# benjisu03/grayshift

Hardware: AMD Instinct MI355X
Metric: Msamples/sec (primary+secondary rays) (higher is better)
Workload: dtype f64; 1 GPU; C4: bouncing_spheres_50 1920x1080, 512 spp; tile=64, parallelism=tiles1, tile_plan=round-robin, collective=none, launch=one process, 1 device(s): gs_multi_create once, gs_multi_render per frame, seed=1, rays_per_frame=2921120250

## Files before the change

__graft_entry__.py:

```python
import os
import sys

ROOT = os.path.dirname(os.path.abspath(__file__))


def build():
    sys.path.insert(0, ROOT)
    from grayshift_amd import build as b
    b.build_product()
    b.build_oracle()
    b.build_kat()
    import grayshift_amd
    from grayshift_amd import _native


def smoke():
    sys.path.insert(0, ROOT)
    sys.path.insert(0, os.path.join(ROOT, "oracle"))
    import numpy as np
    import grayshift_amd as g
    from grayshift_amd import scenes
    import oracle

    sc = scenes.config("C4", width=48, spp=4)
    out, gc = g.render(sc, seed=7)
    ref, rc = oracle.render(sc, seed=7)
    d = float(np.abs(out.astype(np.float64) - ref.astype(np.float64)).max())
    if not (d < 1e-3) or gc != rc:
        raise AssertionError("smoke parity failed: max|d|=%g counters gpu=%s oracle=%s" % (d, gc, rc))
    print("smoke ok: C4 48x27x4spp max|d|=%g rays=%d" % (d, gc["rays"]))


if __name__ == "__main__":
    build()
# ... 3 lines not shown
```

grayshift_amd/build.py:

```python
import argparse
import glob
import os
import subprocess
import sys

HERE = os.path.dirname(os.path.abspath(__file__))
ROOT = os.path.dirname(HERE)
LIB = os.path.join(HERE, "libgrayshift.so")
ORACLE_DIR = os.path.join(ROOT, "oracle")
ORACLE_LIB = os.path.join(ORACLE_DIR, "liboracle.so")

SOURCES = [
    os.path.join(HERE, "csrc", "device", "render.hip"),
    os.path.join(HERE, "csrc", "device", "output.hip"),
    os.path.join(HERE, "csrc", "device", "bvh_build.hip"),
    os.path.join(HERE, "csrc", "host", "scene.cpp"),
    os.path.join(HERE, "csrc", "host", "launch.cpp"),
    os.path.join(HERE, "csrc", "host", "world.cpp"),
    os.path.join(HERE, "csrc", "host", "camera.cpp"),
    os.path.join(HERE, "csrc", "host", "host_capi.cpp"),
    os.path.join(HERE, "csrc", "host", "multi_gpu.cpp"),
]


# ... 45 lines not shown
    if verbose:
        print(" ".join(cmd), flush=True)
    subprocess.run(cmd, check=True)
    os.replace(tmp, lib)
    return lib


KAT_SRC = os.path.join(ROOT, "tests", "hip", "kat_device.hip")
KAT_LIB = os.path.join(ROOT, "tests", "hip", "libkat_device.so")


def build_kat(force=False, verbose=False):
    deps = [KAT_SRC] + _headers()
    if not force and not _stale(KAT_LIB, deps):
        return KAT_LIB
    cmd = [HIPCC] + COMMON + ["-x", "hip", "--offload-arch=" + ARCH, "-shared", "-o", KAT_LIB + ".tmp", KAT_SRC]
    if verbose:
        print(" ".join(cmd), flush=True)
    subprocess.run(cmd, check=True)
    os.replace(KAT_LIB + ".tmp", KAT_LIB)
    return KAT_LIB


def build_oracle(force=False, verbose=False):
    if force and os.path.exists(ORACLE_LIB):
        os.remove(ORACLE_LIB)
    subprocess.run(["make", "-s", "-C", ORACLE_DIR], check=True,
                   stdout=None if verbose else subprocess.DEVNULL)
    return ORACLE_LIB


def main(argv=None):
    ap = argparse.ArgumentParser()
    ap.add_argument("--force", action="store_true")
    ap.add_argument("--no-oracle", action="store_true")
    ap.add_argument("-v", "--verbose", action="store_true")
    ap.add_argument("--variant", action="append", metavar="NAME:FLAGS", default=[],
                    help="also build variants/NAME.so with extra FLAGS (A/B), e.g. --variant 'v4:-DGS_MIN_WAVES=4'")
    ap.add_argument("--resource-usage", action="store_true",
                    help="print per-kernel VGPR/SGPR/LDS/occupancy (hipcc remarks)")
    a = ap.parse_args(argv)
    extra = ["-Rpass-analysis=kernel-resource-usage"] if a.resource_usage else []
    import concurrent.futures as cf

    def variant(spec):
        name, _, flags = spec.partition(":")
        path = os.path.join(HERE, "variants", name + ".so")
        os.makedirs(os.path.dirname(path), exist_ok=True)
        build_product(force=True, verbose=a.verbose, extra=extra + flags.split(), out=path)
        return "variant %s %s" % (path, flags)

    with cf.ThreadPoolExecutor(max_workers=4) as ex:
        jobs = [ex.submit(build_product, force=a.force or a.resource_usage, verbose=a.verbose, extra=extra)]
        jobs += [ex.submit(variant, spec) for spec in a.variant]
        for j in jobs[1:]:
            print(j.result())
        jobs[0].result()
    if not a.no_oracle:
        build_oracle(force=a.force, verbose=a.verbose)
        build_kat(force=a.force, verbose=a.verbose)
    print("built", LIB, "" if a.no_oracle else ORACLE_LIB)


if __name__ == "__main__":
    sys.exit(main())
```

grayshift_amd/csrc/device/devmath.hpp:

```cpp
#pragma once
#include <hip/hip_runtime.h>
#include <stdint.h>

#include "kernel_abi.hpp"

namespace gsd {

struct d3 {
    double x, y, z;
};

__device__ __forceinline__ d3 mk(double x, double y, double z) { return d3{x, y, z}; }
__device__ __forceinline__ d3 add(d3 a, d3 b) { return d3{a.x + b.x, a.y + b.y, a.z + b.z}; }
__device__ __forceinline__ d3 sub(d3 a, d3 b) { return d3{a.x - b.x, a.y - b.y, a.z - b.z}; }
__device__ __forceinline__ d3 neg(d3 a) { return d3{-a.x, -a.y, -a.z}; }
__device__ __forceinline__ d3 muls(d3 a, double s) { return d3{a.x * s, a.y * s, a.z * s}; }
__device__ __forceinline__ d3 mulv(d3 a, d3 b) { return d3{a.x * b.x, a.y * b.y, a.z * b.z}; }
__device__ __forceinline__ d3 divs(d3 a, double s) { return d3{a.x / s, a.y / s, a.z / s}; }
__device__ __forceinline__ double dot(d3 a, d3 b) { return a.x * b.x + a.y * b.y + a.z * b.z; }
__device__ __forceinline__ double len2(d3 a) { return a.x * a.x + a.y * a.y + a.z * a.z; }
__device__ __forceinline__ d3 cross(d3 a, d3 b) {
    return d3{a.y * b.z - a.z * b.y, a.z * b.x - a.x * b.z, a.x * b.y - a.y * b.x};
}
__device__ __forceinline__ d3 unit(d3 a) { return divs(a, sqrt(len2(a))); }
__device__ __forceinline__ d3 reflect(d3 v, d3 n) { return sub(v, muls(n, 2.0 * dot(v, n))); }
__device__ __forceinline__ d3 refract(d3 v, d3 n, double ratio) {
    double cos_theta = fmin(dot(n, neg(v)), 1.0);
    d3 perp = muls(add(v, muls(n, cos_theta)), ratio);
    d3 par = muls(n, -sqrt(fabs(1.0 - len2(perp))));
    return add(perp, par);
}
__device__ __forceinline__ d3 ld3(const double* p) { return d3{p[0], p[1], p[2]}; }

__device__ __forceinline__ uint64_t wy_next(uint64_t& state) {
    const uint64_t C0 = 0x2d358dccaa6c78a5ULL, C1 = 0x8bb84b93962eacc9ULL;
    uint64_t s = state + C0;
    state = s;
    uint64_t b = s ^ C1;
    const uint32_t s0 = (uint32_t)s, s1 = (uint32_t)(s >> 32), b0 = (uint32_t)b, b1 = (uint32_t)(b >> 32);
    const uint64_t p00 = (uint64_t)s0 * b0;
    const uint64_t t = (uint64_t)s0 * b1 + (p00 >> 32);
    const uint64_t u = (uint64_t)s1 * b0 + (uint32_t)t;
    const uint64_t hi = (uint64_t)s1 * b1 + ((t >> 32) + (u >> 32));
    const uint64_t lo = (u << 32) | (uint32_t)p00;
    return lo ^ hi;
}
__device__ __forceinline__ double wy_f64(uint64_t& state) {
    uint64_t bits = 0x3FF0000000000000ULL | (wy_next(state) >> 12);
    return __longlong_as_double((long long)bits) - 1.0;
}
__device__ __forceinline__ uint64_t splitmix64(uint64_t x) {
    uint64_t z = x + 0x9E3779B97F4A7C15ULL;
// ... 34 lines not shown
```

grayshift_amd/csrc/device/geometry.hpp:

```cpp
#pragma once
#include "../../../include/grayshift_gpu.h"
#include "kernel_abi.hpp"
#include "devmath.hpp"

namespace gsd {

struct Ray {
    d3 o, d;
    double time;
};

__device__ __forceinline__ DNode load_node(const DNode* p) {
    const uint4* q = reinterpret_cast<const uint4*>(p);
    const uint4 a = q[0], b = q[1], c = q[2], d = q[3];
    DNode n;
    n.mnx = __hiloint2double((int)a.y, (int)a.x);
    n.mny = __hiloint2double((int)a.w, (int)a.z);
    n.mnz = __hiloint2double((int)b.y, (int)b.x);
    n.mxx = __hiloint2double((int)b.w, (int)b.z);
    n.mxy = __hiloint2double((int)c.y, (int)c.x);
    n.mxz = __hiloint2double((int)c.w, (int)c.z);
    n.left = d.x;
    n.right = d.y;
    n.pad0 = d.z;
// ... 65 lines not shown
}
__device__ __forceinline__ bool box_hit_fast(const DNode& n, const d3& o, const d3& inv, double tmin, double tmax) {
    double hi = tmax;
    double lo;
    {
        const double t0 = (n.mnx - o.x) * inv.x, t1 = (n.mxx - o.x) * inv.x;
        lo = hw_max_u(tmin, hw_min(t0, t1));
        hi = hw_min(hi, hw_max(t0, t1));
    }
    slab_fast(n.mny, n.mxy, o.y, inv.y, lo, hi);
    slab_fast(n.mnz, n.mxz, o.z, inv.z, lo, hi);
    return !(hi <= lo);
}

#define GS_CERT_K 4.76837158203125e-07f

typedef float gs_f2 __attribute__((ext_vector_type(2)));
struct RayCert {
    gs_f2 ixy, oxy;
    gs_f2 izz, ozz;
    float r2;
};

__device__ __forceinline__ double rcp_cert(double d) {
    double r = __builtin_amdgcn_rcp(d);
    double e = __builtin_fma(-d, r, 1.0);
    r = __builtin_fma(r, e, r);
    e = __builtin_fma(-d, r, 1.0);
    return __builtin_fma(r, e, r);
}
__host__ __device__ __forceinline__ bool cert_ray_ok(const d3& o, const d3& inv) {
    auto ok_inv = [](double v) { return __builtin_fabs(v) <= 1e15 && __builtin_fabs(v) >= 1e-25; };
    auto ok_o = [](double v) { return __builtin_fabs(v) <= 1e15; };
    return ok_inv(inv.x) && ok_inv(inv.y) && ok_inv(inv.z) && ok_o(o.x) && ok_o(o.y) && ok_o(o.z);
}
__device__ __forceinline__ RayCert make_cert(const d3& o, const d3& inv) {
    RayCert c;
    const double px = o.x * inv.x, py = o.y * inv.y, pz = o.z * inv.z;
    const double R = __builtin_fmax(__builtin_fabs(px), __builtin_fmax(__builtin_fabs(py), __builtin_fabs(pz)));
    c.ixy = gs_f2{(float)inv.x, (float)inv.y};
    c.oxy = gs_f2{(float)(-px), (float)(-py)};
    c.izz = gs_f2{(float)inv.z, (float)inv.z};
    c.ozz = gs_f2{(float)(-pz), (float)(-pz)};
    c.r2 = (float)(2.0 * (double)GS_CERT_K * R * (1.0 + 0x1p-20)) + 1e-30f;
    return c;
}
__device__ __forceinline__ bool box_cert_dt(float mnx, float mny, float mnz, float mxx, float mxy, float mxz,
                                            const RayCert& c, float tmin32, float closest32, float& d, float& thr) {
    const gs_f2 t0 = __builtin_elementwise_fma(gs_f2{mnx, mny}, c.ixy, c.oxy);
    const gs_f2 t1 = __builtin_elementwise_fma(gs_f2{mxx, mxy}, c.ixy, c.oxy);
    const gs_f2 tz = __builtin_elementwise_fma(gs_f2{mnz, mxz}, c.izz, c.ozz);
    const float t0x = t0.x, t1x = t1.x, t0y = t0.y, t1y = t1.y, t0z = tz.x, t1z = tz.y;
    const float lo = __builtin_fmaxf(__builtin_fmaxf(tmin32, __builtin_fminf(t0x, t1x)),
// ... 36 lines not shown
    if (!(tmin < t && t < tmax)) {
        t = (h + sq) / a;
        if (!(tmin < t && t < tmax)) return false;
    }
    t_out = t;
    return true;
}
__device__ __forceinline__ bool sphere_accept(d3 c, double r, const Ray& ray, double a, double tmin, double tmax,
                                         double& t_out) {
    return sphere_accept_rr(c, r * r, ray, a, tmin, tmax, t_out);
}

struct SphereDisc {
    double h, disc;
};
__device__ __forceinline__ SphereDisc sphere_disc_rr(d3 c, double rr, const Ray& ray, double a) {
    d3 oc = sub(c, ray.o);
    SphereDisc s;
    s.h = dot(ray.d, oc);
    double cc = len2(oc) - rr;
    s.disc = s.h * s.h - a * cc;
    return s;
}
__device__ __forceinline__ bool sphere_root_take(double h, double disc, double a, double tmin, double tmax, double& t_out) {
    double sq = sqrt(disc);
    double t = (h - sq) / a;
    if (!(tmin < t && t < tmax)) {
        t = (h + sq) / a;
        if (!(tmin < t && t < tmax)) return false;
    }
    t_out = t;
    return true;
}

__device__ __forceinline__ double div_by(double num, double den, double rden) {
    const double q = num * rden;
    const double r = __builtin_fma(-den, q, num);
    return __builtin_fma(r, rden, q);
}
__device__ __forceinline__ bool sphere_root_take_ra(double h, double disc, double a, double ra, double tmin, double tmax,
                                                    double& t_out) {
    double sq = sqrt(disc);
    double t = div_by(h - sq, a, ra);
    if (!(tmin < t && t < tmax)) {
        t = div_by(h + sq, a, ra);
        if (!(tmin < t && t < tmax)) return false;
    }
    t_out = t;
    return true;
}

__device__ __forceinline__ bool sphere_accept_rr_ra(d3 c, double rr, const Ray& ray, double a, double ra, double tmin,
                                                    double tmax, double& t_out) {
    d3 oc = sub(c, ray.o);
    double h = dot(ray.d, oc);
    double cc = len2(oc) - rr;
    double disc = h * h - a * cc;
    t_out = tmax;
    if (disc < 0.0) return false;
    return sphere_root_take_ra(h, disc, a, ra, tmin, tmax, t_out);
}

__device__ __forceinline__ void sky_index_f64(d3 rot, uint32_t W, uint32_t H, uint32_t& x, uint32_t& y) {
    const double PI = 3.14159265358979323846;
    double theta = atan2(rot.y, rot.x);
    double phi = asin(rot.z);
    double u = 0.5 + theta / (2.0 * PI);
    double v = 0.5 - phi / PI;
    x = (uint32_t)(sat_u64(u * (double)W, 18446744073709551616.0, ~0ull) % (uint64_t)W);
    y = (uint32_t)(sat_u64(v * (double)H, 18446744073709551616.0, ~0ull) % (uint64_t)H);
}
__device__ __forceinline__ bool sky_index_f32(d3 rot, uint32_t W, uint32_t H, uint32_t& x, uint32_t& y) {
    const float fx = (float)rot.x, fy = (float)rot.y, fz = (float)rot.z;
    const float r = __builtin_sqrtf(__builtin_fmaf(fx, fx, fy * fy));
    const float th = atan2f(fy, fx), ph = atan2f(fz, r);
    const float fW = (float)W, fH = (float)H;
    const float U = __builtin_fmaf(th, fW * 0.159154943f, fW * 0.5f);
    const float V = __builtin_fmaf(ph, fH * -0.318309886f, fH * 0.5f);
    const float iu = __builtin_floorf(U), iv = __builtin_floorf(V);
    const float du = U - iu, dv = V - iv;
    const float mu = fW * 1e-6f, mv = fH * 2e-6f;
    x = (uint32_t)(int32_t)iu;
    y = (uint32_t)(int32_t)iv;
// ... 75 lines not shown
```

grayshift_amd/csrc/device/render.hip:

```cpp

#include <hip/hip_runtime.h>

#include <cstdio>
#include <cmath>
#include <cstring>
#include <type_traits>

#include "../../../include/grayshift_gpu.h"
#include "kernel_abi.hpp"
#include "kernels.hpp"
#include "devmath.hpp"
#include "geometry.hpp"
#include "perlin.hpp"

using namespace gsd;

#ifndef GS_NOINLINE
#define GS_NOINLINE __forceinline__
#endif
#ifndef GS_ROOT_RCP
#define GS_ROOT_RCP 1
#endif
#ifndef GS_PRIO_NODE
#define GS_PRIO_NODE 1
// ... 143 lines not shown
        for (uint32_t k = threadIdx.x; k < A.lds_cubes * (GS_CUBE_DOUBLES / 2); k += GS_BLOCK) dst[k] = src[k];
    }
    uint8_t* s_cubes = s_quads + (size_t)A.lds_quads * sizeof(TQuad);
    const QuadSrc qs{s_quads, A.tquads, A.lds_quads, s_cubes, A.lds_cubes};
    double* s_d = (double*)(s_cubes + (size_t)A.lds_cubes * (GS_CUBE_DOUBLES * 8));
    uint32_t* s_i = (uint32_t*)(s_d + A.lane_nd * GS_BLOCK);
    unsigned long long* s_cnt = (unsigned long long*)(s_i + lane_ni(FEAT) * GS_BLOCK);
#ifdef GS_STAMPS
    unsigned long long* s_reg = s_cnt + 16;
    if (threadIdx.x < (GS_BLOCK / 64) * 16) s_reg[threadIdx.x] = 0;
#endif
    if (threadIdx.x < GS_CNT_SLOTS) s_cnt[threadIdx.x] = 0;
    __syncthreads();

    const KParams* __restrict__ P = A.P;
    const DevScene& sc = P->sc;
    const gs_camera& cam = P->cam;
    const uint32_t lane = threadIdx.x & 63;
    const uint32_t tid = threadIdx.x;
    const uint64_t flushers = __builtin_amdgcn_ballot_w64(tid < GS_CNT_SLOTS);
    const double tmin = 0.001;
    constexpr int kUnroll = unroll_steps(FEAT);
    constexpr bool kSphLeaf = (FEAT & GS_FEAT_SPHLEAF) != 0;
    constexpr bool kFixed = (FEAT & GS_FEAT_FIXED) != 0;
    constexpr bool kRsplit = kFixed && (FEAT & GS_FEAT_RSPLIT) != 0;
    constexpr bool kGeneral = (FEAT & GS_FEAT_GENERAL) != 0;
    constexpr bool kViews = (FEAT & GS_FEAT_VIEWS) != 0;
#define LD(k) s_d[((k) + (t_in_lds(FEAT) ? 3 : 0)) * GS_BLOCK + tid]
#define LI(k) s_i[(k) * GS_BLOCK + tid]
    if constexpr (kSphLeaf) LI(L_HINST) = GS_REF_NONE;
    constexpr bool kNested = (FEAT & GS_FEAT_NESTED) != 0;
    uint32_t ninst_ = GS_REF_NONE;
#define LNINST (*(ninst_in_lds(FEAT) ? &s_i[lane_ninst(FEAT) * GS_BLOCK + tid] : &ninst_))
    if constexpr (kNested) LNINST = GS_REF_NONE;
    double* const s_save = s_d + (size_t)(A.lane_nd - A.nest_lds) * GS_BLOCK + tid;
    const size_t g_lanes = (size_t)gridDim.x * GS_BLOCK;
#define NSAVE(k)                                                                                   \
    (*(nest_save_lds(FEAT) && A.nest_lds ? &s_save[(size_t)(k) * GS_BLOCK]                         \
                                         : &P->nest_save[(size_t)(k) * g_lanes + (size_t)blockIdx.x * GS_BLOCK + tid]))

    uint32_t st = S_NEED;
    bool qdone = false;
    uint32_t res_base = 0, res_cnt = 0;
    uint64_t rng = 0;
    constexpr bool kTLds = t_in_lds(FEAT);
    double Tr_ = 1, Tg_ = 1, Tb_ = 1;
// ... 545 lines not shown
                {
                    const uint64_t act = __builtin_amdgcn_read_exec();
                    const bool first = __builtin_ctzll(act) == (uint32_t)lane;
                    bool bad = false;
                    uint32_t kinds = 0;
                    uint64_t m = act;
                    while (m) {
                        const uint32_t L = (uint32_t)__builtin_ctzll(m);
                        const uint32_t r0 = __builtin_amdgcn_readlane(ref, L);
                        const uint64_t same = __builtin_amdgcn_ballot_w64(ref == r0);
                        bad |= ((same >> L) & 1u) == 0;
                        kinds |= 1u << (r0 >> GS_REF_SHIFT);
                        m &= ~(same | (1ull << L));
                        dist_ref += first;
                    }
                    dist_kind += first ? (uint64_t)__builtin_popcount(kinds) : 0;
                    dist_bad += bad && first;
                }
#endif
                auto sphere_test = [&](d3 c, double rr, double& t) __attribute__((always_inline)) {
                    const double a = len2(ray.d);
                    constexpr bool kRa = GS_ROOT_RCP && (FEAT & (GS_FEAT_MEDIA | GS_FEAT_NESTED)) == 0;
                    if (kRa && __builtin_amdgcn_ballot_w64(!(a >= 0x1p-900 && a <= 0x1p900)) == 0)
                        return sphere_accept_rr_ra(c, rr, ray, a, rcp_cert(a), tmin, closest, t);
                    return sphere_accept_rr(c, rr, ray, a, tmin, closest, t);
                };
                auto sphere_leaf = [&]() __attribute__((always_inline)) {
                    GS_MARK("sphere_begin");
                    count_sph();
                    double t;
                    if (sphere_test(mk(scx, scy, scz), sr, t)) {
                        closest = t;
                        closest32 = (float)t;
                        hit_ref = ref;
                        if constexpr (kNested) LI(L_HINST) = LNINST;
                        else if constexpr (!kSphLeaf) LI(L_HINST) = GS_REF_NONE;
                    }
                    GS_MARK("sphere_end");
                };
                if constexpr ((FEAT & GS_FEAT_SPHLEAF) != 0) {
                    const bool two = cur_next_is_leaf(next);
                    double s2x, s2y, s2z, s2r;
                    uint32_t next2, ref2;
                    load_tleaf<(FEAT & GS_FEAT_LDSTREE) != 0>(s_leaves, A.tleaves, two ? next & ~THR_LEAF : cur & ~THR_LEAF,
                                                             A.lds_leaves, s2x, s2y, s2z, s2r, next2, ref2);
                    const double a = len2(ray.d);
                    const SphereDisc q1 = sphere_disc_rr(mk(scx, scy, scz), sr, ray, a);
// ... 141 lines not shown
        GS_STAMP(ts2);
#ifdef GS_STAMPS
        {
            const uint64_t sm = __builtin_amdgcn_ballot_w64(st == S_SHADE);
            it_shade += sm != 0;
            ln_shade += (uint64_t)__popcll(sm);
        }
#endif
        if (st == S_SHADE) {
            bool ends = true;
            double Lr = 0.0, Lg = 0.0, Lb = 0.0;
#ifdef GS_STAMPS
            uint64_t r0;
#endif
            if constexpr ((FEAT & (GS_FEAT_MIXED | GS_FEAT_MEDIA | GS_FEAT_NESTED)) != 0) {
                GS_STAMP(r0);
                GS_MARK("shade_begin"); GS_PRIO_SET(GS_PRIO_SHADE);
#if defined(GS_DIAG_DUP) && (GS_DIAG_DUP & 1)
                {
                    Ray r2 = ray;
                    uint64_t g2 = rng;
                    double c2 = closest;
                    asm volatile("" : "+v"(r2.d.x), "+v"(c2));
                    const ShadeOut s2 = shade<(FEAT & GS_FEAT_PLAIN) != 0, kSphLeaf, kGeneral>(sc, r2, c2, hit_ref, LI(L_HINST), g2, s_cnt);
                    asm volatile("" ::"v"(s2.col.x), "v"(s2.col.y), "v"(s2.col.z), "v"(s2.dir.x), "v"(s2.dir.y), "v"(s2.dir.z),
                                 "v"(r2.o.x), "v"(g2), "v"(s2.cont));
                }
#endif
                uint32_t hinst = (FEAT & GS_FEAT_PLAIN) ? GS_REF_NONE : LI(L_HINST), houter = GS_REF_NONE;
                if constexpr (kNested && kGeneral) {
                    if (hinst != GS_REF_NONE && (hinst >> 31)) {
                        houter = (uint32_t)__double_as_longlong(NSAVE(7));
                        hinst &= 0x7FFFFFFFu;
                    }
                }
                const ShadeOut s = shade<(FEAT & GS_FEAT_PLAIN) != 0, kSphLeaf, kGeneral>(sc, ray, closest, hit_ref, hinst,
                                                                                        rng, s_cnt, houter);
                GS_MARK("shade_end"); GS_PRIO_CLR(GS_PRIO_SHADE);
                GS_REGION(2, r0);
                if (s.cont) {
                    Tr = Tr * s.col.x;
                    Tg = Tg * s.col.y;
                    Tb = Tb * s.col.z;
                    const uint32_t depth = LI(L_DEPTH) - 1u;
                    LI(L_DEPTH) = depth;
                    if (depth > 0) {
                        ray.d = s.dir;
                        fresh = true;
                        st = S_TRACE;
                        ends = false;
                    }
                } else {
                    Lr = Tr * s.col.x;
                    Lg = Tg * s.col.y;
                    Lb = Tb * s.col.z;
                }
            } else {
                if (hit_ref == GS_REF_NONE) {
                    GS_STAMP(r0);
                    const d3 bg = background(sc, ray.d, s_cnt);
                    GS_REGION(0, r0);
                    Lr = Tr * bg.x;
                    Lg = Tg * bg.y;
                    Lb = Tb * bg.z;
                } else {
                    atomicAdd(&s_cnt[C_HITS], 1ull);
                    GS_STAMP(r0);
                    const HitRec h = kSphLeaf ? reconstruct_sphere<true>(sc, ray, closest, hit_ref)
                                              : reconstruct<false>(sc, ray, closest, hit_ref, LI(L_HINST));
                    GS_REGION(1, r0);
                    GS_STAMP(r0);
                    const Scatter s = scatter(sc, h, ray.d, rng, s_cnt);
                    GS_REGION(2, r0);
                    rng = s.rng;
                    if (s.cont) {
                        Tr = Tr * s.col.x;
                        Tg = Tg * s.col.y;
                        Tb = Tb * s.col.z;
                        const uint32_t depth = LI(L_DEPTH) - 1u;
                        LI(L_DEPTH) = depth;
                        if (depth > 0) {
                            ray.o = h.p;
                            ray.d = s.dir;
                            fresh = true;
                            st = S_TRACE;
                            ends = false;
                        }
                    } else {
                        Lr = Tr * s.col.x;
                        Lg = Tg * s.col.y;
                        Lb = Tb * s.col.z;
                    }
                }
            }
            if (ends) {
// ... 264 lines not shown
```

grayshift_amd/csrc/device/shading.hpp:

```cpp
#pragma once
#include <hip/hip_runtime.h>

#include <cmath>
#include <cstdint>

#include "../../../include/grayshift_gpu.h"
#include "kernel_abi.hpp"
#include "devmath.hpp"
#include "geometry.hpp"
#include "perlin.hpp"

#ifndef GS_NOINLINE
#define GS_NOINLINE __forceinline__
#endif

struct HitRec {
    d3 p, n;
    double u, v;
    uint32_t mat;
    bool front;
};

__device__ __forceinline__ void sphere_uv(d3 p, double& u, double& v) {
    const double PI = 3.14159265358979323846;
    double theta = acos(-p.y);
    double phi = atan2(-p.z, p.x) + PI;
    u = phi / (2.0 * PI);
    v = theta / PI;
}

__device__ __forceinline__ uint32_t chain_at(const DevScene& sc, uint32_t outer, uint32_t inner, int n) {
    uint32_t cur = outer != GS_REF_NONE ? outer : inner;
    bool in_outer = outer != GS_REF_NONE;
#pragma unroll 1
    for (int k = 0; k < 2 * GS_MAX_CHAIN; k++) {
        if ((cur >> GS_REF_SHIFT) != GS_REF_INSTANCE) {
            if (!in_outer) break;
            in_outer = false;
            cur = inner;
            k--;
            continue;
        }
        if (n-- == 0) return cur & GS_REF_MASK;
        cur = sc.inst[cur & GS_REF_MASK].child;
    }
    return 0u;
}
template <bool DEEP>
__device__ GS_NOINLINE HitRec reconstruct(const DevScene& sc, Ray r, double t, uint32_t hit_ref,
                                           uint32_t hit_inst, uint32_t outer = GS_REF_NONE) {
    HitRec h;
    uint32_t ch0 = 0, ch1 = 0, ch2 = 0, ch3 = 0;
    int nch = 0;
    bool deep = DEEP && outer != GS_REF_NONE;
    if (hit_inst != GS_REF_NONE && !deep) {
        uint32_t cur = hit_inst;
#pragma unroll
        for (int k = 0; k < 4; k++) {
            if ((cur >> GS_REF_SHIFT) != GS_REF_INSTANCE) break;
            uint32_t i = cur & GS_REF_MASK;
            if (k == 0) ch0 = i; else if (k == 1) ch1 = i; else if (k == 2) ch2 = i; else ch3 = i;
            nch = k + 1;
            const gs_instance& in = sc.inst[i];
            inst_forward(in, r);
            cur = in.child;
        }
        if (DEEP && (cur >> GS_REF_SHIFT) == GS_REF_INSTANCE) {
            deep = true;
#pragma unroll 1
            for (int k = 4; k < GS_MAX_CHAIN && (cur >> GS_REF_SHIFT) == GS_REF_INSTANCE; k++) {
                const gs_instance& in = sc.inst[cur & GS_REF_MASK];
// ... 17 lines not shown
            inst_forward(in, r);
            cur = in.child;
            nch++;
        }
    }
    const uint32_t kind = hit_ref >> GS_REF_SHIFT, idx = hit_ref & GS_REF_MASK;
    d3 p, outward;
    double u = 0.0, v = 0.0;
    if (kind == GS_REF_SPHERE || kind == GS_REF_MSPHERE) {
        d3 c;
        double rad;
        if (kind == GS_REF_SPHERE) {
            DSphere s = sc.spheres[idx];
            c = mk(s.cx, s.cy, s.cz);
            rad = s.r;
            h.mat = sc.sphere_mat[idx];
        } else {
            const gs_msphere& s = sc.mspheres[idx];
            c = add(ld3(s.center_start), muls(ld3(s.center_path), r.time));
            rad = s.radius;
            h.mat = s.material;
        }
        p = add(r.o, muls(r.d, t));
        outward = divs(sub(p, c), rad);
        if (sc.mats[h.mat].needs_uv) sphere_uv(outward, u, v);
    } else if (kind == GS_REF_QUAD) {
        const gs_quad& q = sc.quads[idx];
        p = add(r.o, muls(r.d, t));
        d3 planar = sub(p, ld3(q.q));
        u = dot(ld3(q.w), cross(planar, ld3(q.v)));
        v = dot(ld3(q.w), cross(ld3(q.u), planar));
        outward = ld3(q.normal);
        h.mat = q.material;
    } else if (kind == GS_REF_MEDIUM) {
        p = add(r.o, muls(r.d, t));
        outward = mk(1.0, 0.0, 0.0);
        h.mat = sc.media[idx].material;
    } else {
        const gs_triangle& tr = sc.tris[idx];
        double tt;
        tri_hit(tr, r, tt, u, v);
        p = add(r.o, muls(r.d, t));
        outward = ld3(tr.normal);
        h.mat = tr.material;
    }
    h.front = dot(r.d, outward) < 0.0;
    d3 n = h.front ? outward : neg(outward);
// ... 64 lines not shown
        const uint8_t* px = sc.texels + im.offset + (j * (uint64_t)im.width + i) * 3;
        atomicAdd(&cnt[C_IMG], 1ull);
        return muls(mk((double)px[0], (double)px[1], (double)px[2]), 1.0 / 255.0);
    }
    return mk(0.0, 0.0, 0.0);
}

__device__ __forceinline__ d3 hdri_texel(const DevScene& sc, d3 rot, unsigned long long* cnt) {
    const gs_background& bg = sc.bg;
    uint32_t x, y;
    if (!sky_index_f32(rot, bg.width, bg.height, x, y)) sky_index_f64(rot, bg.width, bg.height, x, y);
    const uint64_t k = y * (uint64_t)bg.width + x;
    atomicAdd(&cnt[C_HDRI], 1ull);
    if (sc.hdri_rgbe) {
        const uint32_t t = sc.hdri_rgbe[k];
        const uint32_t e = t >> 24;
        const double sc2 = e ? ldexp(1.0, (int)e - 136) : 0.0;
        return mk((double)(t & 0xffu) * sc2, (double)((t >> 8) & 0xffu) * sc2, (double)((t >> 16) & 0xffu) * sc2);
    }
    const float* px = sc.hdri + k * 3;
    return mk((double)px[0], (double)px[1], (double)px[2]);
}

__device__ __forceinline__ d3 checker(const DMaterial& m, d3 p) {
    int32_t xi = sat_i32(floor(m.param * p.x));
    int32_t yi = sat_i32(floor(m.param * p.y));
    int32_t zi = sat_i32(floor(m.param * p.z));
    int32_t s = (int32_t)((uint32_t)xi + (uint32_t)yi + (uint32_t)zi);
    return (s % 2 == 0) ? ld3(m.a) : ld3(m.b);
}

struct ShadeOut {
    d3 col, dir;
    uint32_t cont;
};

template <bool PLAIN, bool SPH, bool GEN>
__device__ __forceinline__ ShadeOut shade(const DevScene& sc, Ray& ray, double t, uint32_t hit_ref,
                                          uint32_t hit_inst, uint64_t& rng, unsigned long long* cnt,
                                          uint32_t hit_outer = GS_REF_NONE) {
    const double PI = 3.14159265358979323846;
    ShadeOut o;
    o.cont = 0;
    o.col = mk(0.0, 0.0, 0.0);
    o.dir = mk(0.0, 0.0, 0.0);
    const bool miss = hit_ref == GS_REF_NONE;
    HitRec h;
    h.p = h.n = mk(0.0, 0.0, 0.0);
    h.u = h.v = 0.0;
    h.front = false;
    uint32_t kind = 0;
    const DMaterial* m = sc.mats;
    if (!miss) {
        atomicAdd(&cnt[C_HITS], 1ull);
        h = PLAIN ? reconstruct_sphere<false>(sc, ray, t, hit_ref)
            : SPH ? reconstruct_sphere<true>(sc, ray, t, hit_ref) : reconstruct<GEN>(sc, ray, t, hit_ref, hit_inst, hit_outer);
        m = &sc.mats[h.mat];
        kind = m->kind;
        ray.o = h.p;
    }
    const bool lamb = kind >= DM_LAMB_SOLID && kind <= DM_LAMB_TEX;
    const bool metal = kind == DM_METAL;
    const bool diel = kind == DM_DIELECTRIC;
    const bool iso = !PLAIN && (kind == DM_ISO_SOLID || kind == DM_ISO_TEX);
    const bool sky = miss && sc.bg.kind != GS_BG_SOLID;

    if (!PLAIN && (kind == DM_LAMB_TEX || kind == DM_LIGHT_TEX || kind == DM_ISO_TEX)) {
        o.col = texture_value(sc, m->texture, h.u, h.v, h.p, cnt);
    } else if (kind == DM_LAMB_CHECKER) {
        o.col = checker(*m, h.p);
    } else if (kind == DM_DIELECTRIC) {
        o.col = mk(1.0, 1.0, 1.0);
    } else if (!miss) {
        o.col = ld3(m->a);
    } else if (!sky) {
        o.col = ld3(sc.bg.color);
    }

    d3 v1 = mk(1.0, 0.0, 0.0);
    if (sky) {
        const double* R = sc.bg.rot;
        const d3 dir = ray.d;
        v1 = mk(dir.x * R[0] + dir.y * R[1] + dir.z * R[2], dir.x * R[3] + dir.y * R[4] + dir.z * R[5],
                dir.x * R[6] + dir.y * R[7] + dir.z * R[8]);
    } else if (lamb) {
        v1 = h.n;
    } else if (metal) {
        v1 = reflect(ray.d, h.n);
    } else if (diel) {
        v1 = ray.d;
    }
    const d3 u1 = unit(v1);

    d3 v2 = mk(1.0, 0.0, 0.0);
    double q2 = 1.0, ri = 0.0, cos_theta = 0.0;
    if (sky) {
        o.col = hdri_texel(sc, u1, cnt);
    } else if (lamb) {
        const d3 a = fabs(u1.x) > 0.9 ? mk(0.0, 1.0, 0.0) : mk(1.0, 0.0, 0.0);
        v2 = cross(u1, a);
        q2 = len2(v2);
    } else if (metal || iso) {
#pragma unroll 1
        for (;;) {
            double x = wy_f64(rng) * 2.0 + -1.0;
            double y = wy_f64(rng) * 2.0 + -1.0;
            double z = wy_f64(rng) * 2.0 + -1.0;
            v2 = mk(x, y, z);
            q2 = len2(v2);
            if (q2 < 1.0) break;
        }
    } else if (diel) {
        ri = h.front ? 1.0 / m->param : m->param;
        cos_theta = fmin(dot(neg(u1), h.n), 1.0);
        q2 = 1.0 - cos_theta * cos_theta;
    }
    const double r2v = sqrt(q2);
    d3 u2 = v2;
    if (lamb || metal || iso) u2 = divs(v2, r2v);

    double rd = 0.0;
    if (lamb || diel) rd = wy_f64(rng);
    d3 w3 = mk(0.0, 0.0, 0.0), n3 = h.n;
    double q3 = 1.0;
    bool third = false;
    if (lamb) {
        const d3 vv = u2;
        const d3 uu = cross(u1, vv);
        double r1 = rd;
        double r2 = wy_f64(rng);
        double phi = 2.0 * PI * r1;
        double r2s = sqrt(r2);
        double sp, cp;
        sincos(phi, &sp, &cp);
        double q = sqrt(r2s);
        d3 cd = mk(cp * q, sp * q, sqrt(1.0 - r2));
        w3 = add(add(muls(uu, cd.x), muls(vv, cd.y)), muls(u1, cd.z));
        q3 = len2(w3);
        third = true;
        o.cont = 1;
    } else if (metal) {
        const d3 reflected = add(u1, muls(u2, m->param));
        if (dot(reflected, h.n) > 0.0) {
            o.dir = reflected;
            o.cont = 1;
        } else {
            o.col = mk(0.0, 0.0, 0.0);
        }
    } else if (iso) {
        o.dir = u2;
        o.cont = 1;
    } else if (diel) {
        const d3 ud = u1;
        double sin_theta = r2v;
        bool cannot_refract = ri * sin_theta > 1.0;
        double r0 = (1.0 - ri) / (1.0 + ri);
        r0 = r0 * r0;
        double x = 1.0 - cos_theta;
        double x2 = x * x;
        double x4 = x2 * x2;
        double refl = r0 + (1.0 - r0) * (x * x4);
        bool fresnel = refl > rd;
        if (cannot_refract || fresnel) {
            o.dir = reflect(ud, h.n);
        } else {
            double ct = fmin(dot(h.n, neg(ud)), 1.0);
            w3 = muls(add(ud, muls(h.n, ct)), ri);
            q3 = fabs(1.0 - len2(w3));
            third = true;
        }
        o.cont = 1;
    }
    if (third) {
        const double r3 = sqrt(q3);
        if (lamb) o.dir = divs(w3, r3);
        else o.dir = add(w3, muls(n3, -r3));
    }
    return o;
}

__device__ GS_NOINLINE d3 background(const DevScene& sc, d3 dir, unsigned long long* cnt) {
    const gs_background& bg = sc.bg;
    if (bg.kind == GS_BG_SOLID) return ld3(bg.color);
    d3 rv = mk(dir.x * bg.rot[0] + dir.y * bg.rot[1] + dir.z * bg.rot[2],
               dir.x * bg.rot[3] + dir.y * bg.rot[4] + dir.z * bg.rot[5],
               dir.x * bg.rot[6] + dir.y * bg.rot[7] + dir.z * bg.rot[8]);
    return hdri_texel(sc, unit(rv), cnt);
}

__device__ __forceinline__ d3 random_unit_vector(uint64_t& rng) {
    d3 v;
#pragma unroll 1
    for (;;) {
        double x = wy_f64(rng) * 2.0 + -1.0;
        double y = wy_f64(rng) * 2.0 + -1.0;
        double z = wy_f64(rng) * 2.0 + -1.0;
        v = mk(x, y, z);
        if (len2(v) < 1.0) break;
    }
    return unit(v);
}

struct Scatter {
    d3 col, dir;
    uint64_t rng;
    uint32_t cont;
};

__device__ GS_NOINLINE Scatter scatter(const DevScene& sc, HitRec h, d3 in_dir, uint64_t rng,
                                        unsigned long long* cnt) {
    const DMaterial& m = sc.mats[h.mat];
    Scatter s;
    s.cont = 0;
    s.col = mk(0.0, 0.0, 0.0);
    s.dir = mk(0.0, 0.0, 0.0);
    const uint32_t kind = m.kind;
    if (kind <= DM_LAMB_TEX) {
        s.col = kind == DM_LAMB_SOLID ? ld3(m.a)
              : kind == DM_LAMB_CHECKER ? checker(m, h.p)
                                        : texture_value(sc, m.texture, h.u, h.v, h.p, cnt);
        d3 w = unit(h.n);
        d3 a = fabs(w.x) > 0.9 ? mk(0.0, 1.0, 0.0) : mk(1.0, 0.0, 0.0);
        d3 vv = unit(cross(w, a));
        d3 uu = cross(w, vv);
        const double PI = 3.14159265358979323846;
        double r1 = wy_f64(rng);
        double r2 = wy_f64(rng);
        double phi = 2.0 * PI * r1;
        double r2s = sqrt(r2);
        double sp, cp;
        sincos(phi, &sp, &cp);
        double q = sqrt(r2s);
        d3 cd = mk(cp * q, sp * q, sqrt(1.0 - r2));
        s.dir = unit(add(add(muls(uu, cd.x), muls(vv, cd.y)), muls(w, cd.z)));
        s.cont = 1;
    } else if (kind == DM_METAL) {
        d3 reflected = reflect(in_dir, h.n);
        reflected = add(unit(reflected), muls(random_unit_vector(rng), m.param));
        if (dot(reflected, h.n) > 0.0) {
            s.col = ld3(m.a);
            s.dir = reflected;
            s.cont = 1;
        }
    } else if (kind == DM_DIELECTRIC) {
        double ri = h.front ? 1.0 / m.param : m.param;
        d3 ud = unit(in_dir);
        double cos_theta = fmin(dot(neg(ud), h.n), 1.0);
        double sin_theta = sqrt(1.0 - cos_theta * cos_theta);
        bool cannot_refract = ri * sin_theta > 1.0;
        double r0 = (1.0 - ri) / (1.0 + ri);
        r0 = r0 * r0;
        double x = 1.0 - cos_theta;
        double x2 = x * x;
        double x4 = x2 * x2;
        double refl = r0 + (1.0 - r0) * (x * x4);
        bool fresnel = refl > wy_f64(rng);
        s.dir = (cannot_refract || fresnel) ? reflect(ud, h.n) : refract(ud, h.n, ri);
        s.col = mk(1.0, 1.0, 1.0);
        s.cont = 1;
    } else if (kind == DM_ISO_SOLID || kind == DM_ISO_TEX) {
        s.col = kind == DM_ISO_SOLID ? ld3(m.a) : texture_value(sc, m.texture, h.u, h.v, h.p, cnt);
        s.dir = random_unit_vector(rng);
        s.cont = 1;
    } else {
        s.col = kind == DM_LIGHT_SOLID ? ld3(m.a) : texture_value(sc, m.texture, h.u, h.v, h.p, cnt);
    }
    s.rng = rng;
    return s;
}
```

grayshift_amd/csrc/host/scene.cpp:

```cpp
#include <algorithm>
#include <cmath>
#include <cstring>
#include <functional>
#include <memory>
#include <unordered_map>

#include "render_host.hpp"

using namespace gsd;

namespace {

#ifndef GS_LDS_MIRROR
#define GS_LDS_MIRROR -1
#endif
const int64_t g_lds_mirror = GS_LDS_MIRROR;
int64_t lds_mirror_budget() {
    const int64_t share = (int64_t)160 * 1024 * GS_BLOCK / (GS_MIN_WAVES * 4 * 64);
    const int64_t left = share - (int64_t)GS_BLOCK * (L_ND_CHUNKED * 8 + L_NI * 4) - 1024;
    return left > 0 ? left : 0;
}
#ifndef GS_KIND_SHADE_BATCH
#define GS_KIND_SHADE_BATCH 44
#endif
// ... 615 lines not shown
            if (m.kind == GS_MAT_LAMBERTIAN) {
                d.kind = solid ? DM_LAMB_SOLID : (checker2 ? DM_LAMB_CHECKER : DM_LAMB_TEX);
            } else if (m.kind == GS_MAT_ISOTROPIC) {
                d.kind = solid ? DM_ISO_SOLID : DM_ISO_TEX;
            } else {
                d.kind = solid ? DM_LIGHT_SOLID : DM_LIGHT_TEX;
            }
            if (solid) {
                for (int k = 0; k < 3; k++) d.a[k] = t.color[k];
            } else if (checker2 && m.kind == GS_MAT_LAMBERTIAN) {
                for (int k = 0; k < 3; k++) {
                    d.a[k] = s.textures[t.even].color[k];
                    d.b[k] = s.textures[t.odd].color[k];
                }
                d.param = t.scale_inv;
            }
        } else if (m.kind == GS_MAT_METAL) {
            d.kind = DM_METAL;
            for (int k = 0; k < 3; k++) d.a[k] = m.albedo[k];
            d.param = m.param;
        } else {
            d.kind = DM_DIELECTRIC;
            d.param = m.param;
        }
        mats[i] = d;
    }
    return mats;
}

struct FeatFacts {
    bool media;
    bool nested;
    bool general;
    bool leaf_runs;
    bool sph_leaves;
    bool all_mirrored;
    bool sky;
    const std::vector<DMaterial>* mats;
};
int choose_feat(const FeatFacts& f) {
    if (f.general) return GS_FEAT_GENERAL_KERNEL;
    int feat = (f.media ? GS_FEAT_MEDIA : 0) | (f.nested ? GS_FEAT_NESTED : 0) | (f.leaf_runs ? GS_FEAT_LEAFRUN : 0);
    const bool flat = !(feat & (GS_FEAT_MEDIA | GS_FEAT_NESTED));
    if (flat && f.all_mirrored) feat |= GS_FEAT_LDSTREE;
    bool lamb = false, metal = false, diel = false, iso = false;
    for (const DMaterial& m : *f.mats) {
// ... 228 lines not shown
```

Measured before the change: 8930 Msamples/s.

## Replace f64 sqrt/div with wave-guarded correctly-rounded rsq/rcp Newton sequences

Adds fast paths for f64 sqrt, vector division and normalisation. They use the hardware rsq/rcp approximations refined by FMA Newton steps, so one reciprocal is shared across the three components. A wave-wide ballot range check falls back to library sqrt/div when any lane has an out-of-range operand. Dielectric constants (1/ior and squared Fresnel r0 for both faces) are also precomputed on the host into material slots. The aim is to cut the long f64 division and sqrt sequences in shading and sphere intersection while keeping bit-exact results, at the cost of extra ballots and branches.

```diff
diff --git a/__graft_entry__.py b/__graft_entry__.py
--- a/__graft_entry__.py
+++ b/__graft_entry__.py
@@ -10,6 +10,7 @@
     b.build_product()
     b.build_oracle()
     b.build_kat()
+    b.build_kat_exact()
     import grayshift_amd
     from grayshift_amd import _native
 
diff --git a/grayshift_amd/build.py b/grayshift_amd/build.py
--- a/grayshift_amd/build.py
+++ b/grayshift_amd/build.py
@@ -91,6 +91,23 @@
     return KAT_LIB
 
 
+KAT_EXACT_SRC = os.path.join(ROOT, "tests", "hip", "kat_exact.hip")
+KAT_EXACT_LIB = os.path.join(ROOT, "tests", "hip", "libkat_exact.so")
+
+
+def build_kat_exact(force=False, verbose=False):
+    deps = [KAT_EXACT_SRC] + _headers()
+    if not force and not _stale(KAT_EXACT_LIB, deps):
+        return KAT_EXACT_LIB
+    cmd = [HIPCC] + COMMON + ["-x", "hip", "--offload-arch=" + ARCH, "-shared", "-o", KAT_EXACT_LIB + ".tmp",
+                              KAT_EXACT_SRC]
+    if verbose:
+        print(" ".join(cmd), flush=True)
+    subprocess.run(cmd, check=True)
+    os.replace(KAT_EXACT_LIB + ".tmp", KAT_EXACT_LIB)
+    return KAT_EXACT_LIB
+
+
 def build_oracle(force=False, verbose=False):
     if force and os.path.exists(ORACLE_LIB):
         os.remove(ORACLE_LIB)
@@ -128,6 +145,7 @@
     if not a.no_oracle:
         build_oracle(force=a.force, verbose=a.verbose)
         build_kat(force=a.force, verbose=a.verbose)
+        build_kat_exact(force=a.force, verbose=a.verbose)
     print("built", LIB, "" if a.no_oracle else ORACLE_LIB)
 
 
diff --git a/grayshift_amd/csrc/device/devmath.hpp b/grayshift_amd/csrc/device/devmath.hpp
--- a/grayshift_amd/csrc/device/devmath.hpp
+++ b/grayshift_amd/csrc/device/devmath.hpp
@@ -16,18 +16,119 @@
 __device__ __forceinline__ d3 neg(d3 a) { return d3{-a.x, -a.y, -a.z}; }
 __device__ __forceinline__ d3 muls(d3 a, double s) { return d3{a.x * s, a.y * s, a.z * s}; }
 __device__ __forceinline__ d3 mulv(d3 a, d3 b) { return d3{a.x * b.x, a.y * b.y, a.z * b.z}; }
-__device__ __forceinline__ d3 divs(d3 a, double s) { return d3{a.x / s, a.y / s, a.z / s}; }
 __device__ __forceinline__ double dot(d3 a, d3 b) { return a.x * b.x + a.y * b.y + a.z * b.z; }
 __device__ __forceinline__ double len2(d3 a) { return a.x * a.x + a.y * a.y + a.z * a.z; }
 __device__ __forceinline__ d3 cross(d3 a, d3 b) {
     return d3{a.y * b.z - a.z * b.y, a.z * b.x - a.x * b.z, a.x * b.y - a.y * b.x};
 }
-__device__ __forceinline__ d3 unit(d3 a) { return divs(a, sqrt(len2(a))); }
+
+#ifndef GS_VDIV_SHARED
+#define GS_VDIV_SHARED 1
+#endif
+#ifndef GS_SQRT_DIRECT
+#define GS_SQRT_DIRECT 1
+#endif
+#define GS_EXACT_LO 0x1p-250
+#define GS_EXACT_HI 0x1p250
+__device__ __forceinline__ int exact_in(double v) {
+    return (int)(__builtin_fabs(v) >= GS_EXACT_LO) & (int)(__builtin_fabs(v) <= GS_EXACT_HI);
+}
+__device__ __forceinline__ int exact_in0(double v) { return (int)(v == 0.0) | exact_in(v); }
+__device__ __forceinline__ int exact_lo0(double v) { return (int)(v == 0.0) | (int)(__builtin_fabs(v) >= GS_EXACT_LO); }
+__device__ __forceinline__ bool wave_all(int ok) { return __builtin_amdgcn_ballot_w64(ok == 0) == 0; }
+#define GS_LIKELY(c) __builtin_expect((c), 1)
+
+__device__ __forceinline__ double rcp_cert(double d) {
+    double r = __builtin_amdgcn_rcp(d);
+    double e = __builtin_fma(-d, r, 1.0);
+    r = __builtin_fma(r, e, r);
+    e = __builtin_fma(-d, r, 1.0);
+    return __builtin_fma(r, e, r);
+}
+__device__ __forceinline__ double div_by(double num, double den, double rden) {
+    const double q = num * rden;
+    const double r = __builtin_fma(-den, q, num);
+    return __builtin_fma(r, rden, q);
+}
+__device__ __forceinline__ double div_by_signed(double num, double den, double rden) {
+    const double q = num * rden;
+    const double r = __builtin_fma(-den, q, num);
+    return __builtin_copysign(__builtin_fma(r, rden, q), q);
+}
+__device__ __forceinline__ double sqrt_seq(double x) {
+    const double y = __builtin_amdgcn_rsq(x);
+    double g = x * y;
+    double h = y * 0.5;
+    const double r = __builtin_fma(-h, g, 0.5);
+    g = __builtin_fma(g, r, g);
+    h = __builtin_fma(h, r, h);
+    double d = __builtin_fma(-g, g, x);
+    g = __builtin_fma(d, h, g);
+    d = __builtin_fma(-g, g, x);
+    return __builtin_fma(d, h, g);
+}
+__device__ __forceinline__ d3 div3_plain(d3 a, double s) { return d3{a.x / s, a.y / s, a.z / s}; }
+__device__ __forceinline__ d3 div3_by(d3 a, double s, double rs) {
+    return d3{div_by_signed(a.x, s, rs), div_by_signed(a.y, s, rs), div_by_signed(a.z, s, rs)};
+}
+
+__device__ __forceinline__ double sqrt_direct(double x, bool& fast) {
+    fast = GS_SQRT_DIRECT && wave_all((int)(x >= GS_EXACT_LO) & (int)(x <= GS_EXACT_HI));
+    if (GS_LIKELY(fast)) return sqrt_seq(x);
+    return sqrt(x);
+}
+__device__ __forceinline__ d3 div3_shared(d3 a, double s, bool& fast) {
+    fast = GS_VDIV_SHARED && wave_all(exact_in(s) & exact_in0(a.x) & exact_in0(a.y) & exact_in0(a.z));
+    if (GS_LIKELY(fast)) return div3_by(a, s, rcp_cert(s));
+    return div3_plain(a, s);
+}
+__device__ __forceinline__ d3 unit_shared(d3 a, bool& fast) {
+    const double l = len2(a);
+    if (GS_VDIV_SHARED && GS_SQRT_DIRECT) {
+        fast = wave_all(exact_in(l) & exact_lo0(a.x) & exact_lo0(a.y) & exact_lo0(a.z));
+        if (GS_LIKELY(fast)) {
+            const double s = sqrt_seq(l);
+            return div3_by(a, s, rcp_cert(s));
+        }
+        return div3_plain(a, sqrt(l));
+    }
+    bool f;
+    const double s = sqrt_direct(l, f);
+    return div3_shared(a, s, fast);
+}
+template <bool EX = true>
+__device__ __forceinline__ double sqrt_x(double x) {
+    if constexpr (EX) {
+        bool f;
+        return sqrt_direct(x, f);
+    } else {
+        return sqrt(x);
+    }
+}
+template <bool EX = true>
+__device__ __forceinline__ d3 divs(d3 a, double s) {
+    if constexpr (EX) {
+        bool f;
+        return div3_shared(a, s, f);
+    } else {
+        return div3_plain(a, s);
+    }
+}
+template <bool EX = true>
+__device__ __forceinline__ d3 unit(d3 a) {
+    if constexpr (EX) {
+        bool f;
+        return unit_shared(a, f);
+    } else {
+        return div3_plain(a, sqrt(len2(a)));
+    }
+}
 __device__ __forceinline__ d3 reflect(d3 v, d3 n) { return sub(v, muls(n, 2.0 * dot(v, n))); }
+template <bool EX = true>
 __device__ __forceinline__ d3 refract(d3 v, d3 n, double ratio) {
     double cos_theta = fmin(dot(n, neg(v)), 1.0);
     d3 perp = muls(add(v, muls(n, cos_theta)), ratio);
-    d3 par = muls(n, -sqrt(fabs(1.0 - len2(perp))));
+    d3 par = muls(n, -sqrt_x<EX>(fabs(1.0 - len2(perp))));
     return add(perp, par);
 }
 __device__ __forceinline__ d3 ld3(const double* p) { return d3{p[0], p[1], p[2]}; }
diff --git a/grayshift_amd/csrc/device/geometry.hpp b/grayshift_amd/csrc/device/geometry.hpp
--- a/grayshift_amd/csrc/device/geometry.hpp
+++ b/grayshift_amd/csrc/device/geometry.hpp
@@ -111,13 +111,6 @@
     float r2;
 };
 
-__device__ __forceinline__ double rcp_cert(double d) {
-    double r = __builtin_amdgcn_rcp(d);
-    double e = __builtin_fma(-d, r, 1.0);
-    r = __builtin_fma(r, e, r);
-    e = __builtin_fma(-d, r, 1.0);
-    return __builtin_fma(r, e, r);
-}
 __host__ __device__ __forceinline__ bool cert_ray_ok(const d3& o, const d3& inv) {
     auto ok_inv = [](double v) { return __builtin_fabs(v) <= 1e15 && __builtin_fabs(v) >= 1e-25; };
     auto ok_o = [](double v) { return __builtin_fabs(v) <= 1e15; };
@@ -200,8 +193,9 @@
     s.disc = s.h * s.h - a * cc;
     return s;
 }
+template <bool EX = true>
 __device__ __forceinline__ bool sphere_root_take(double h, double disc, double a, double tmin, double tmax, double& t_out) {
-    double sq = sqrt(disc);
+    double sq = sqrt_x<EX>(disc);
     double t = (h - sq) / a;
     if (!(tmin < t && t < tmax)) {
         t = (h + sq) / a;
@@ -211,14 +205,10 @@
     return true;
 }
 
-__device__ __forceinline__ double div_by(double num, double den, double rden) {
-    const double q = num * rden;
-    const double r = __builtin_fma(-den, q, num);
-    return __builtin_fma(r, rden, q);
-}
+template <bool EX = true>
 __device__ __forceinline__ bool sphere_root_take_ra(double h, double disc, double a, double ra, double tmin, double tmax,
                                                     double& t_out) {
-    double sq = sqrt(disc);
+    double sq = sqrt_x<EX>(disc);
     double t = div_by(h - sq, a, ra);
     if (!(tmin < t && t < tmax)) {
         t = div_by(h + sq, a, ra);
@@ -228,6 +218,7 @@
     return true;
 }
 
+template <bool EX = true>
 __device__ __forceinline__ bool sphere_accept_rr_ra(d3 c, double rr, const Ray& ray, double a, double ra, double tmin,
                                                     double tmax, double& t_out) {
     d3 oc = sub(c, ray.o);
@@ -236,7 +227,7 @@
     double disc = h * h - a * cc;
     t_out = tmax;
     if (disc < 0.0) return false;
-    return sphere_root_take_ra(h, disc, a, ra, tmin, tmax, t_out);
+    return sphere_root_take_ra<EX>(h, disc, a, ra, tmin, tmax, t_out);
 }
 
 __device__ __forceinline__ void sky_index_f64(d3 rot, uint32_t W, uint32_t H, uint32_t& x, uint32_t& y) {
diff --git a/grayshift_amd/csrc/device/render.hip b/grayshift_amd/csrc/device/render.hip
--- a/grayshift_amd/csrc/device/render.hip
+++ b/grayshift_amd/csrc/device/render.hip
@@ -189,6 +189,7 @@
     const double tmin = 0.001;
     constexpr int kUnroll = unroll_steps(FEAT);
     constexpr bool kSphLeaf = (FEAT & GS_FEAT_SPHLEAF) != 0;
+    constexpr bool kExact = kSphLeaf || ((FEAT & GS_FEAT_MIXED) != 0 && (FEAT & (GS_FEAT_MEDIA | GS_FEAT_NESTED)) == 0);
     constexpr bool kFixed = (FEAT & GS_FEAT_FIXED) != 0;
     constexpr bool kRsplit = kFixed && (FEAT & GS_FEAT_RSPLIT) != 0;
     constexpr bool kGeneral = (FEAT & GS_FEAT_GENERAL) != 0;
@@ -780,7 +781,7 @@
                     const double a = len2(ray.d);
                     constexpr bool kRa = GS_ROOT_RCP && (FEAT & (GS_FEAT_MEDIA | GS_FEAT_NESTED)) == 0;
                     if (kRa && __builtin_amdgcn_ballot_w64(!(a >= 0x1p-900 && a <= 0x1p900)) == 0)
-                        return sphere_accept_rr_ra(c, rr, ray, a, rcp_cert(a), tmin, closest, t);
+                        return sphere_accept_rr_ra<kExact>(c, rr, ray, a, rcp_cert(a), tmin, closest, t);
                     return sphere_accept_rr(c, rr, ray, a, tmin, closest, t);
                 };
                 auto sphere_leaf = [&]() __attribute__((always_inline)) {
@@ -968,7 +969,7 @@
                     uint64_t g2 = rng;
                     double c2 = closest;
                     asm volatile("" : "+v"(r2.d.x), "+v"(c2));
-                    const ShadeOut s2 = shade<(FEAT & GS_FEAT_PLAIN) != 0, kSphLeaf, kGeneral>(sc, r2, c2, hit_ref, LI(L_HINST), g2, s_cnt);
+                    const ShadeOut s2 = shade<(FEAT & GS_FEAT_PLAIN) != 0, kSphLeaf, kGeneral, kExact>(sc, r2, c2, hit_ref, LI(L_HINST), g2, s_cnt);
                     asm volatile("" ::"v"(s2.col.x), "v"(s2.col.y), "v"(s2.col.z), "v"(s2.dir.x), "v"(s2.dir.y), "v"(s2.dir.z),
                                  "v"(r2.o.x), "v"(g2), "v"(s2.cont));
                 }
@@ -980,7 +981,7 @@
                         hinst &= 0x7FFFFFFFu;
                     }
                 }
-                const ShadeOut s = shade<(FEAT & GS_FEAT_PLAIN) != 0, kSphLeaf, kGeneral>(sc, ray, closest, hit_ref, hinst,
+                const ShadeOut s = shade<(FEAT & GS_FEAT_PLAIN) != 0, kSphLeaf, kGeneral, kExact>(sc, ray, closest, hit_ref, hinst,
                                                                                         rng, s_cnt, houter);
                 GS_MARK("shade_end"); GS_PRIO_CLR(GS_PRIO_SHADE);
                 GS_REGION(2, r0);
@@ -1004,7 +1005,7 @@
             } else {
                 if (hit_ref == GS_REF_NONE) {
                     GS_STAMP(r0);
-                    const d3 bg = background(sc, ray.d, s_cnt);
+                    const d3 bg = background<kExact>(sc, ray.d, s_cnt);
                     GS_REGION(0, r0);
                     Lr = Tr * bg.x;
                     Lg = Tg * bg.y;
@@ -1013,10 +1014,10 @@
                     atomicAdd(&s_cnt[C_HITS], 1ull);
                     GS_STAMP(r0);
                     const HitRec h = kSphLeaf ? reconstruct_sphere<true>(sc, ray, closest, hit_ref)
-                                              : reconstruct<false>(sc, ray, closest, hit_ref, LI(L_HINST));
+                                              : reconstruct<false, kExact>(sc, ray, closest, hit_ref, LI(L_HINST));
                     GS_REGION(1, r0);
                     GS_STAMP(r0);
-                    const Scatter s = scatter(sc, h, ray.d, rng, s_cnt);
+                    const Scatter s = scatter<kExact>(sc, h, ray.d, rng, s_cnt);
                     GS_REGION(2, r0);
                     rng = s.rng;
                     if (s.cont) {
diff --git a/grayshift_amd/csrc/device/shading.hpp b/grayshift_amd/csrc/device/shading.hpp
--- a/grayshift_amd/csrc/device/shading.hpp
+++ b/grayshift_amd/csrc/device/shading.hpp
@@ -46,7 +46,7 @@
     }
     return 0u;
 }
-template <bool DEEP>
+template <bool DEEP, bool EX = true>
 __device__ GS_NOINLINE HitRec reconstruct(const DevScene& sc, Ray r, double t, uint32_t hit_ref,
                                            uint32_t hit_inst, uint32_t outer = GS_REF_NONE) {
     HitRec h;
@@ -110,7 +110,7 @@
             h.mat = s.material;
         }
         p = add(r.o, muls(r.d, t));
-        outward = divs(sub(p, c), rad);
+        outward = divs<EX>(sub(p, c), rad);
         if (sc.mats[h.mat].needs_uv) sphere_uv(outward, u, v);
     } else if (kind == GS_REF_QUAD) {
         const gs_quad& q = sc.quads[idx];
@@ -221,6 +221,20 @@
     return mk((double)px[0], (double)px[1], (double)px[2]);
 }
 
+#ifndef GS_DIEL_CONST
+#define GS_DIEL_CONST 1
+#endif
+template <bool EX = true>
+__device__ __forceinline__ double diel_inv(const DMaterial& m) {
+    return GS_DIEL_CONST && EX ? m.b[0] : 1.0 / m.param;
+}
+template <bool EX = true>
+__device__ __forceinline__ double diel_r0sq(const DMaterial& m, bool front, double ri) {
+    if (GS_DIEL_CONST && EX) return front ? m.b[1] : m.b[2];
+    const double r0 = (1.0 - ri) / (1.0 + ri);
+    return r0 * r0;
+}
+
 __device__ __forceinline__ d3 checker(const DMaterial& m, d3 p) {
     int32_t xi = sat_i32(floor(m.param * p.x));
     int32_t yi = sat_i32(floor(m.param * p.y));
@@ -234,7 +248,7 @@
     uint32_t cont;
 };
 
-template <bool PLAIN, bool SPH, bool GEN>
+template <bool PLAIN, bool SPH, bool GEN, bool EX = true>
 __device__ __forceinline__ ShadeOut shade(const DevScene& sc, Ray& ray, double t, uint32_t hit_ref,
                                           uint32_t hit_inst, uint64_t& rng, unsigned long long* cnt,
                                           uint32_t hit_outer = GS_REF_NONE) {
@@ -253,7 +267,7 @@
     if (!miss) {
         atomicAdd(&cnt[C_HITS], 1ull);
         h = PLAIN ? reconstruct_sphere<false>(sc, ray, t, hit_ref)
-            : SPH ? reconstruct_sphere<true>(sc, ray, t, hit_ref) : reconstruct<GEN>(sc, ray, t, hit_ref, hit_inst, hit_outer);
+            : SPH ? reconstruct_sphere<true>(sc, ray, t, hit_ref) : reconstruct<GEN, EX>(sc, ray, t, hit_ref, hit_inst, hit_outer);
         m = &sc.mats[h.mat];
         kind = m->kind;
         ray.o = h.p;
@@ -289,7 +303,7 @@
     } else if (diel) {
         v1 = ray.d;
     }
-    const d3 u1 = unit(v1);
+    const d3 u1 = unit<EX>(v1);
 
     d3 v2 = mk(1.0, 0.0, 0.0);
     double q2 = 1.0, ri = 0.0, cos_theta = 0.0;
@@ -310,13 +324,13 @@
             if (q2 < 1.0) break;
         }
     } else if (diel) {
-        ri = h.front ? 1.0 / m->param : m->param;
+        ri = h.front ? diel_inv<EX>(*m) : m->param;
         cos_theta = fmin(dot(neg(u1), h.n), 1.0);
         q2 = 1.0 - cos_theta * cos_theta;
     }
-    const double r2v = sqrt(q2);
+    const double r2v = sqrt_x<EX>(q2);
     d3 u2 = v2;
-    if (lamb || metal || iso) u2 = divs(v2, r2v);
+    if (lamb || metal || iso) u2 = divs<EX>(v2, r2v);
 
     double rd = 0.0;
     if (lamb || diel) rd = wy_f64(rng);
@@ -329,11 +343,11 @@
         double r1 = rd;
         double r2 = wy_f64(rng);
         double phi = 2.0 * PI * r1;
-        double r2s = sqrt(r2);
+        double r2s = sqrt_x<EX>(r2);
         double sp, cp;
         sincos(phi, &sp, &cp);
-        double q = sqrt(r2s);
-        d3 cd = mk(cp * q, sp * q, sqrt(1.0 - r2));
+        double q = sqrt_x<EX>(r2s);
+        d3 cd = mk(cp * q, sp * q, sqrt_x<EX>(1.0 - r2));
         w3 = add(add(muls(uu, cd.x), muls(vv, cd.y)), muls(u1, cd.z));
         q3 = len2(w3);
         third = true;
@@ -353,8 +367,7 @@
         const d3 ud = u1;
         double sin_theta = r2v;
         bool cannot_refract = ri * sin_theta > 1.0;
-        double r0 = (1.0 - ri) / (1.0 + ri);
-        r0 = r0 * r0;
+        const double r0 = diel_r0sq<EX>(*m, h.front, ri);
         double x = 1.0 - cos_theta;
         double x2 = x * x;
         double x4 = x2 * x2;
@@ -371,22 +384,24 @@
         o.cont = 1;
     }
     if (third) {
-        const double r3 = sqrt(q3);
-        if (lamb) o.dir = divs(w3, r3);
+        const double r3 = sqrt_x<EX>(q3);
+        if (lamb) o.dir = divs<EX>(w3, r3);
         else o.dir = add(w3, muls(n3, -r3));
     }
     return o;
 }
 
+template <bool EX = true>
 __device__ GS_NOINLINE d3 background(const DevScene& sc, d3 dir, unsigned long long* cnt) {
     const gs_background& bg = sc.bg;
     if (bg.kind == GS_BG_SOLID) return ld3(bg.color);
     d3 rv = mk(dir.x * bg.rot[0] + dir.y * bg.rot[1] + dir.z * bg.rot[2],
                dir.x * bg.rot[3] + dir.y * bg.rot[4] + dir.z * bg.rot[5],
                dir.x * bg.rot[6] + dir.y * bg.rot[7] + dir.z * bg.rot[8]);
-    return hdri_texel(sc, unit(rv), cnt);
-}
-
+    return hdri_texel(sc, unit<EX>(rv), cnt);
+}
+
+template <bool EX = true>
 __device__ __forceinline__ d3 random_unit_vector(uint64_t& rng) {
     d3 v;
 #pragma unroll 1
@@ -397,7 +412,7 @@
         v = mk(x, y, z);
         if (len2(v) < 1.0) break;
     }
-    return unit(v);
+    return unit<EX>(v);
 }
 
 struct Scatter {
@@ -406,6 +421,7 @@
     uint32_t cont;
 };
 
+template <bool EX = true>
 __device__ GS_NOINLINE Scatter scatter(const DevScene& sc, HitRec h, d3 in_dir, uint64_t rng,
                                         unsigned long long* cnt) {
     const DMaterial& m = sc.mats[h.mat];
@@ -418,48 +434,47 @@
         s.col = kind == DM_LAMB_SOLID ? ld3(m.a)
               : kind == DM_LAMB_CHECKER ? checker(m, h.p)
                                         : texture_value(sc, m.texture, h.u, h.v, h.p, cnt);
-        d3 w = unit(h.n);
+        d3 w = unit<EX>(h.n);
         d3 a = fabs(w.x) > 0.9 ? mk(0.0, 1.0, 0.0) : mk(1.0, 0.0, 0.0);
-        d3 vv = unit(cross(w, a));
+        d3 vv = unit<EX>(cross(w, a));
         d3 uu = cross(w, vv);
         const double PI = 3.14159265358979323846;
         double r1 = wy_f64(rng);
         double r2 = wy_f64(rng);
         double phi = 2.0 * PI * r1;
-        double r2s = sqrt(r2);
+        double r2s = sqrt_x<EX>(r2);
         double sp, cp;
         sincos(phi, &sp, &cp);
-        double q = sqrt(r2s);
-        d3 cd = mk(cp * q, sp * q, sqrt(1.0 - r2));
-        s.dir = unit(add(add(muls(uu, cd.x), muls(vv, cd.y)), muls(w, cd.z)));
+        double q = sqrt_x<EX>(r2s);
+        d3 cd = mk(cp * q, sp * q, sqrt_x<EX>(1.0 - r2));
+        s.dir = unit<EX>(add(add(muls(uu, cd.x), muls(vv, cd.y)), muls(w, cd.z)));
         s.cont = 1;
     } else if (kind == DM_METAL) {
         d3 reflected = reflect(in_dir, h.n);
-        reflected = add(unit(reflected), muls(random_unit_vector(rng), m.param));
+        reflected = add(unit<EX>(reflected), muls(random_unit_vector<EX>(rng), m.param));
         if (dot(reflected, h.n) > 0.0) {
             s.col = ld3(m.a);
             s.dir = reflected;
             s.cont = 1;
         }
     } else if (kind == DM_DIELECTRIC) {
-        double ri = h.front ? 1.0 / m.param : m.param;
-        d3 ud = unit(in_dir);
+        double ri = h.front ? diel_inv<EX>(m) : m.param;
+        d3 ud = unit<EX>(in_dir);
         double cos_theta = fmin(dot(neg(ud), h.n), 1.0);
-        double sin_theta = sqrt(1.0 - cos_theta * cos_theta);
+        double sin_theta = sqrt_x<EX>(1.0 - cos_theta * cos_theta);
         bool cannot_refract = ri * sin_theta > 1.0;
-        double r0 = (1.0 - ri) / (1.0 + ri);
-        r0 = r0 * r0;
+        const double r0 = diel_r0sq<EX>(m, h.front, ri);
         double x = 1.0 - cos_theta;
         double x2 = x * x;
         double x4 = x2 * x2;
         double refl = r0 + (1.0 - r0) * (x * x4);
         bool fresnel = refl > wy_f64(rng);
-        s.dir = (cannot_refract || fresnel) ? reflect(ud, h.n) : refract(ud, h.n, ri);
+        s.dir = (cannot_refract || fresnel) ? reflect(ud, h.n) : refract<EX>(ud, h.n, ri);
         s.col = mk(1.0, 1.0, 1.0);
         s.cont = 1;
     } else if (kind == DM_ISO_SOLID || kind == DM_ISO_TEX) {
         s.col = kind == DM_ISO_SOLID ? ld3(m.a) : texture_value(sc, m.texture, h.u, h.v, h.p, cnt);
-        s.dir = random_unit_vector(rng);
+        s.dir = random_unit_vector<EX>(rng);
         s.cont = 1;
     } else {
         s.col = kind == DM_LIGHT_SOLID ? ld3(m.a) : texture_value(sc, m.texture, h.u, h.v, h.p, cnt);
diff --git a/grayshift_amd/csrc/host/scene.cpp b/grayshift_amd/csrc/host/scene.cpp
--- a/grayshift_amd/csrc/host/scene.cpp
+++ b/grayshift_amd/csrc/host/scene.cpp
@@ -661,6 +661,11 @@
         } else {
             d.kind = DM_DIELECTRIC;
             d.param = m.param;
+            const double inv = 1.0 / m.param;
+            const double r0f = (1.0 - inv) / (1.0 + inv), r0b = (1.0 - m.param) / (1.0 + m.param);
+            d.b[0] = inv;
+            d.b[1] = r0f * r0f;
+            d.b[2] = r0b * r0b;
         }
         mats[i] = d;
     }
```

After: 8973 Msamples/s, median of 6. Within noise of the previous version (+0.5%).
